# ga1i13o/DiffewS

Hardware: AMD Instinct MI355X
Metric: few-shot episodes/sec (512x512, 1-shot, SD-2 UNet) (higher is better)
Workload: dtype bf16; 1 GPU; SD-2.1 UNet + SD VAE, 512x512, 1-shot, 4 episodes/GPU/step (BASELINE.json configs[1]); nshot=1, resolution=512, parallelism=episode-sharded x1, hip_graph=True, residual_dtype=bf16, graph_owner=pipeline.run_episodes(captured=True)

## Files before the change

diffews_amd/_lib.py:

```python
import ctypes as C
import os

_HERE = os.path.dirname(os.path.abspath(__file__))
LIB_PATH = os.environ.get("DFW_LIB") or os.path.join(_HERE, "libdiffews_hip.so")

BF16, F16 = 0, 1
FILTER_BILINEAR, FILTER_BICUBIC = 0, 1
OUT_T, OUT_F32, OUT_NCHW_F32 = 0, 1, 2
ACT_NONE, ACT_SILU, ACT_CLAMP1 = 0, 1, 2

_vp, _i32, _i64, _f32, _sz = C.c_void_p, C.c_int32, C.c_int64, C.c_float, C.c_size_t


class GemmArgs(C.Structure):
    _fields_ = [("A", _vp), ("W", _vp), ("C", _vp), ("bias", _vp), ("rowbias", _vp), ("residual", _vp),
                ("workspace", _vp), ("workspace_bytes", _sz), ("a_elems", _i64), ("w_elems", _i64),
                ("M", _i32), ("N", _i32), ("K", _i32), ("lda", _i32), ("ldc", _i32), ("ldr", _i32), ("ld_rowbias", _i32),
                ("taps", _i32), ("Cin", _i32), ("Hi", _i32), ("Wi", _i32), ("Ho", _i32), ("Wo", _i32),
                ("stride", _i32), ("pad", _i32), ("ups", _i32), ("rows_per_img", _i32),
                ("out_scale", _f32), ("act", _i32), ("geglu", _i32), ("out_mode", _i32), ("splitk", _i32),
                ("batch", _i32), ("strideA", _i64), ("strideW", _i64), ("strideC", _i64), ("dtype", _i32),
                ("gn_partial", _vp), ("gn_groups", _i32),
                ("colscale", _f32), ("colscale_n", _i32), ("residual_f32", _i32), ("W_blocked", _vp)]


class FsaArgs(C.Structure):
    _fields_ = [("q", _vp), ("k", _vp), ("v", _vp), ("k_bank", _vp), ("v_bank", _vp), ("out", _vp),
                ("batch", _i32), ("heads", _i32), ("n_q", _i32), ("n_kv", _i32), ("n_bank", _i32), ("nshot", _i32),
                ("ldq", _i32), ("ldk", _i32), ("ldv", _i32), ("ldkb", _i32), ("ldvb", _i32), ("ldo", _i32),
                ("q_bs", _i64), ("k_bs", _i64), ("v_bs", _i64), ("kb_bs", _i64), ("vb_bs", _i64), ("o_bs", _i64),
                ("scale", _f32), ("dtype", _i32), ("n_plain", _i32), ("q_prescaled", _i32), ("lse", _vp),
                ("workspace", _vp), ("workspace_bytes", _sz), ("bank_shared", _i32)]


class XattnArgs(C.Structure):
    _fields_ = [("q", _vp), ("k", _vp), ("v", _vp), ("out", _vp),
                ("batch", _i32), ("heads", _i32), ("n_q", _i32), ("L", _i32),
                ("ldq", _i32), ("ldk", _i32), ("ldv", _i32), ("ldo", _i32),
                ("q_bs", _i64), ("k_bs", _i64), ("v_bs", _i64), ("o_bs", _i64),
                ("scale", _f32), ("dtype", _i32)]


class GroupNormArgs(C.Structure):
    _fields_ = [("x", _vp), ("y", _vp), ("gamma", _vp), ("beta", _vp), ("stats_ws", _vp), ("stats_ws_bytes", _sz),
                ("B", _i32), ("HW", _i32), ("C", _i32), ("groups", _i32), ("ldx", _i32), ("ldy", _i32),
                ("eps", _f32), ("silu", _i32), ("dtype", _i32), ("pre_partial", _vp), ("pre_chunks", _i32),
                ("x_f32", _i32)]


class LayerNormArgs(C.Structure):
    _fields_ = [("x", _vp), ("y", _vp), ("gamma", _vp), ("beta", _vp),
                ("rows", _i32), ("C", _i32), ("ldx", _i32), ("ldy", _i32), ("eps", _f32), ("dtype", _i32),
                ("x_f32", _i32)]


class ConvSmallArgs(C.Structure):
    _fields_ = [("x", _vp), ("W", _vp), ("bias", _vp), ("y", _vp),
                ("B", _i32), ("Cin", _i32), ("H", _i32), ("Wd", _i32), ("Cout", _i32), ("taps", _i32), ("ldy", _i32),
                ("in_scale", _f32), ("out_scale", _f32), ("out_mode", _i32), ("dtype", _i32),
                ("gn_partial", _vp), ("gn_groups", _i32), ("y_bstride", _i64),
                ("x1", _vp), ("x2", _vp), ("b0", _i32), ("b1", _i32)]


class ImageArgs(C.Structure):
    _fields_ = [("src", _vp), ("H", _i32), ("W", _i32), ("out_h", _i32), ("out_w", _i32),
                ("xbounds", _vp), ("xcoef", _vp), ("xk", _i32), ("ybounds", _vp), ("ycoef", _vp), ("yk", _i32),
                ("tmp", _vp), ("dst", _vp), ("lut", _vp)]


class NativeItem(C.Structure):
    _fields_ = [("h", _i32), ("w", _i32), ("xk", _i32), ("yk", _i32),
                ("xb_off", _i64), ("xc_off", _i64), ("yb_off", _i64), ("yc_off", _i64),
                ("tmp_off", _i64), ("u8_off", _i64), ("pred_off", _i64), ("gt_off", _i64),
                ("gt_elem", _i32), ("class_value", _i32), ("ignore_value", _i32), ("reserved", _i32)]


class SegNativeArgs(C.Structure):
    _fields_ = [("seg_u8", _vp), ("B", _i32), ("Hs", _i32), ("Ws", _i32), ("items", _vp), ("items_host", _vp),
                ("weights", _vp), ("weights_bytes", _sz), ("gt", _vp), ("gt_bytes", _sz), ("tmp", _vp), ("tmp_bytes", _sz),
                ("tmp_res_off", _sz), ("out_u8", _vp), ("out_u8_bytes", _sz), ("pred", _vp), ("pred_bytes", _sz),
                ("mx", _vp), ("counts", _vp), ("r_threshold", _f32), ("threshold", _f32), ("batch_max", _i32)]


class SegLabelsNativeArgs(C.Structure):
    _fields_ = [("seg_u8", _vp), ("N", _i32), ("B", _i32), ("Hs", _i32), ("Ws", _i32), ("items", _vp), ("items_host", _vp),
                ("weights", _vp), ("weights_bytes", _sz), ("gt", _vp), ("gt_bytes", _sz), ("tmp", _vp), ("tmp_bytes", _sz),
                ("tmp_res_off", _sz), ("tmp_cls_stride", _sz), ("u8_cls_stride", _sz), ("out_u8", _vp), ("out_u8_bytes", _sz),
                ("labels", _vp), ("labels_bytes", _sz), ("mx", _vp), ("counts", _vp), ("class_ids", _vp),
                ("r_threshold", _f32), ("threshold", _f32), ("batch_max", _i32)]


class InputImageItem(C.Structure):
    _fields_ = [("H", _i32), ("W", _i32), ("xk", _i32), ("yk", _i32), ("src_off", _i64),
                ("xb_off", _i64), ("xc_off", _i64), ("yb_off", _i64), ("yc_off", _i64), ("tmp_off", _i64), ("dst_off", _i64)]


class InputMaskItem(C.Structure):
    _fields_ = [("H", _i32), ("W", _i32), ("elem", _i32), ("class_value", _i32),
                ("src_off", _i64), ("pm1_off", _i64), ("bin_off", _i64)]


class InputsArgs(C.Structure):
    _fields_ = [("image_items", _vp), ("image_items_host", _vp), ("n_img", _i32),
                ("mask_items", _vp), ("mask_items_host", _vp), ("n_mask", _i32), ("out_h", _i32), ("out_w", _i32),
                ("staged", _vp), ("staged_bytes", _sz), ("tmp", _vp), ("tmp_bytes", _sz), ("dst", _vp), ("dst_bytes", _sz),
                ("pm1", _vp), ("pm1_bytes", _sz), ("bin", _vp), ("bin_bytes", _sz), ("lut", _vp)]
# ... 41 lines not shown
class AttnBwdArgs(C.Structure):
    _fields_ = [("q", _vp), ("k", _vp), ("v", _vp), ("out", _vp), ("dout", _vp), ("lse", _vp), ("delta", _vp),
                ("dq", _vp), ("dk", _vp), ("dv", _vp),
                ("batch", _i32), ("heads", _i32), ("n_q", _i32), ("n_kv", _i32),
                ("ldq", _i32), ("ldkv", _i32), ("ldo", _i32), ("lddq", _i32), ("lddkv", _i32),
                ("q_bs", _i64), ("kv_bs", _i64), ("o_bs", _i64), ("dq_bs", _i64), ("dkv_bs", _i64),
                ("scale", _f32), ("dtype", _i32), ("workspace", _vp), ("workspace_bytes", _sz), ("delta_bytes", _sz)]


class VattnArgs(C.Structure):
    _fields_ = [("q", _vp), ("k", _vp), ("v", _vp), ("out", _vp),
                ("batch", _i32), ("n", _i32), ("head_dim", _i32), ("q_prescaled", _i32),
                ("ldq", _i32), ("ldk", _i32), ("ldv", _i32), ("ldo", _i32),
                ("q_bs", _i64), ("k_bs", _i64), ("v_bs", _i64), ("o_bs", _i64), ("dtype", _i32)]


class AdamWArgs(C.Structure):
    _fields_ = [("param", _vp), ("grad", _vp), ("exp_avg", _vp), ("exp_avg_sq", _vp), ("grad_sumsq", _vp), ("n", _i64),
                ("lr", _f32), ("beta1", _f32), ("beta2", _f32), ("eps", _f32), ("weight_decay", _f32), ("max_grad_norm", _f32),
                ("step", _i32), ("shadow", _vp), ("shadow_dtype", _i32), ("found_inf", _vp)]


class Config(C.Structure):
    _fields_ = [("conv_patch", _i32), ("big_kernels", _i32), ("big_bm", _i32), ("big_bn", _i32), ("big_bk", _i32),
                ("gemm_bm", _i32), ("gemm_bn", _i32), ("fsa_key_split", _i32),
                ("fsa_force_splits", _i32), ("big_min_tiles", _i32), ("k8", _i32)]


SYMBOLS = {
    "dfw_configure": (_i32, [C.POINTER(Config)]),
    "dfw_get_config": (None, [C.POINTER(Config)]),
    "dfw_version": (_i32, []),
    "dfw_error_string": (C.c_char_p, [_i32]),
    "dfw_graph_memset_nodes": (_i32, [_vp, C.POINTER(_i32)]),
    "dfw_gemm": (_i32, [C.POINTER(GemmArgs), _vp]),
    "dfw_gemm_workspace_bytes": (_sz, [C.POINTER(GemmArgs)]),
    "dfw_gemm_kernel_name": (_i32, [C.POINTER(GemmArgs), C.c_char_p, _sz]),
    "dfw_gemm_gn_chunks": (_i32, [C.POINTER(GemmArgs)]),
    "dfw_fsa_attention": (_i32, [C.POINTER(FsaArgs), _vp]),
    "dfw_fsa_workspace_bytes": (_sz, [C.POINTER(FsaArgs)]),
    "dfw_fsa_kernel_name": (_i32, [C.POINTER(FsaArgs), C.c_char_p, _sz]),
    "dfw_fsa_attention_sets": (_i32, [C.POINTER(FsaArgs), _i32, _vp]),
    "dfw_fsa_sets_kernel_name": (_i32, [C.POINTER(FsaArgs), _i32, C.c_char_p, _sz]),
    "dfw_cross_attention": (_i32, [C.POINTER(XattnArgs), _vp]),
    "dfw_vae_attention": (_i32, [C.POINTER(VattnArgs), _vp]),
    "dfw_groupnorm": (_i32, [C.POINTER(GroupNormArgs), _vp]),
    "dfw_groupnorm_workspace_bytes": (_sz, [C.POINTER(GroupNormArgs)]),
    "dfw_layernorm": (_i32, [C.POINTER(LayerNormArgs), _vp]),
    "dfw_conv_small": (_i32, [C.POINTER(ConvSmallArgs), _vp]),
    "dfw_conv_small_gn_chunks": (_i32, [C.POINTER(ConvSmallArgs)]),
    "dfw_conv_small_kernel_name": (_i32, [C.POINTER(ConvSmallArgs), C.c_char_p, _sz]),
    "dfw_softmax_rows": (_i32, [_vp, _vp, _i64, _i32, _f32, _i32, _vp]),
    "dfw_softmax_groups": (_i32, [_vp, _vp, _i64, _i32, _i32, _i32, _i32, _vp]),
    "dfw_transpose": (_i32, [_vp, _vp, _i32, _i32, _i32, _i32, _vp]),
    "dfw_concat_channels": (_i32, [_vp, _vp, _vp, _i64, _i32, _i32, _i32, _vp]),
    "dfw_convert_f32": (_i32, [_vp, _vp, _i64, _i32, _vp]),
    "dfw_zero": (_i32, [_vp, _i64, _vp]),
    "dfw_split_f32": (_i32, [_vp, _vp, _vp, _i64, _i32, _vp]),
    "dfw_timestep_embedding": (_i32, [_vp, _vp, _i32, _i32, _i32, _f32, _i32, _vp]),
    "dfw_seg_postprocess": (_i32, [_vp, _vp, _vp, _vp, _vp, _i32, _i32, _i32, _f32, _vp]),
    "dfw_seg_postprocess_ex": (_i32, [_vp, _vp, _vp, _vp, _vp, _i32, _i32, _i32, _f32, _f32, _i32, _vp]),
    "dfw_seg_labels": (_i32, [_vp, _vp, _vp, _vp, _vp, _i32, _i32, _i32, _i32, _f32, _f32, _i32, _vp]),
    "dfw_meter_update": (_i32, [_vp, _vp, _vp, _vp, _i32, _i32, _vp]),
    "dfw_gemm_tn": (_i32, [C.POINTER(GemmTnArgs), _vp]),
    "dfw_gemm_tn_workspace_bytes": (_sz, [C.POINTER(GemmTnArgs)]),
    "dfw_gemm_tn_kernel_name": (_i32, [C.POINTER(GemmTnArgs), C.c_char_p, _sz]),
    "dfw_colsum": (_i32, [_vp, _vp, _vp, _sz, _i64, _i32, _i32, _i32, _i64, _f32, _i32, _i32, _vp]),
    "dfw_colsum_plan": (_i32, [_i64, C.POINTER(_i32), C.POINTER(_i32)]),
    "dfw_table_write": (_i32, [_vp, _i64, _vp, _i32, _vp]),
    "dfw_colsum_batch": (_i32, [_vp, _i32, _i64, _i64, _vp, _i32, _vp]),
    "dfw_colsum_workspace_bytes": (_sz, [_i64, _i32, _i32]),
    "dfw_groupnorm_bwd": (_i32, [C.POINTER(GroupNormBwdArgs), _vp]),
    "dfw_groupnorm_bwd_workspace_bytes": (_sz, [C.POINTER(GroupNormBwdArgs)]),
    "dfw_layernorm_bwd": (_i32, [C.POINTER(LayerNormBwdArgs), _vp]),
    "dfw_layernorm_bwd_workspace_bytes": (_sz, [_i32, _i32]),
    "dfw_geglu": (_i32, [_vp, _vp, _vp, _i64, _i32, _i32, _vp]),
    "dfw_elementwise": (_i32, [_i32, _vp, _vp, _vp, _i64, _i32, _i32, _i32, _i32, _i32, _i32, _vp]),
    "dfw_nchw_to_nhwc": (_i32, [_vp, _vp, _i32, _i32, _i32, _i32, _f32, _i32, _vp]),
    "dfw_mse_loss": (_i32, [_vp, _vp, _vp, _vp, _vp, _vp, _i32, _i32, _i32, _f32, _i32, _vp]),
    "dfw_loss_grad": (_i32, [_vp, _vp, _vp, _i32, _i32, _i32, _f32, _i32, _vp]),
    "dfw_convert_to_f32": (_i32, [_vp, _vp, _i64, _f32, _i32, _vp]),
    "dfw_fsa_attention_bwd": (_i32, [C.POINTER(FsaBwdArgs), _vp]),
    "dfw_fsa_attention_bwd_workspace_bytes": (_sz, [C.POINTER(FsaBwdArgs)]),
    "dfw_attention_bwd": (_i32, [C.POINTER(AttnBwdArgs), _vp]),
    "dfw_attention_bwd_workspace_bytes": (_sz, [C.POINTER(AttnBwdArgs)]),
    "dfw_cross_attention_bwd": (_i32, [C.POINTER(XattnBwdArgs), _vp]),
    "dfw_cross_attention_bwd_workspace_bytes": (_sz, [_i32, _i32, _i32, _i32]),
    "dfw_silu": (_i32, [_vp, _vp, _vp, _i64, _i32, _vp]),
    "dfw_sumsq": (_i32, [_vp, _vp, _vp, _i64, _vp]),
    "dfw_adamw": (_i32, [C.POINTER(AdamWArgs), _vp]),
    "dfw_weight_relayout": (_i32, [_vp, _vp, _i32, _i32, _i64, _i64, _i32, _i64, _i64, _i32, _vp]),
    "dfw_weight_relayout_batch": (_i32, [_vp, _i32, _i64, _vp]),
    "dfw_resample_ksize": (_i32, [_i32, _i32]),
    "dfw_resample_coeffs": (_i32, [_i32, _i32, _vp, _vp]),
    "dfw_image_to_tensor": (_i32, [C.POINTER(ImageArgs), _vp]),
    "dfw_mask_to_tensor": (_i32, [_vp, _i32, _i32, _i32, _i32, _i32, _i32, _vp, _vp, _vp]),
    "dfw_resample_ksize_ex": (_i32, [_i32, _i32, _i32]),
    "dfw_resample_coeffs_ex": (_i32, [_i32, _i32, _i32, _vp, _vp]),
    "dfw_seg_native": (_i32, [C.POINTER(SegNativeArgs), _vp]),
    "dfw_seg_labels_native": (_i32, [C.POINTER(SegLabelsNativeArgs), _vp]),
    "dfw_inputs_to_tensor": (_i32, [C.POINTER(InputsArgs), _vp]),
}

_lib = None


# ... 37 lines not shown
```

diffews_amd/build.py:

```python
import os
import subprocess
import sys

HERE = os.path.dirname(os.path.abspath(__file__))
CSRC = os.path.join(HERE, "csrc")
LIB = os.path.join(HERE, "libdiffews_hip.so")
SOURCES = ["gemm.hip", "gemm_big.hip", "gemm8.hip", "conv_patch.hip", "conv_patch8.hip", "attention.hip", "vae_attention.hip", "attention_bwd.hip", "backward.hip", "norm.hip",
           "misc.hip", "inputs.hip", "seg_native.hip"]
FLAGS = ["--offload-arch=gfx950", "-O3", "-std=c++17", "-fPIC", "-ffp-contract=fast", "-Wno-unused-result", "-Wno-unused-value"]


def _src_hash():
    import hashlib
    h = hashlib.sha256(" ".join(FLAGS).encode())
    deps = sorted(os.path.join(CSRC, f) for f in os.listdir(CSRC)) + [os.path.join(HERE, "..", "include", "diffews_hip.h")]
    for d in deps:
        with open(d, "rb") as f:
            h.update(os.path.basename(d).encode() + b"\0" + f.read())
    return h.hexdigest()


def _stale():
    if not os.path.isfile(LIB) or not os.path.isfile(LIB + ".srchash"):
        return True
    with open(LIB + ".srchash") as f:
        return f.read().strip() != _src_hash()


def build(force=False, verbose=False):
    if not force and not _stale():
        return LIB
    if os.environ.get("DFW_NO_BUILD"):
        raise RuntimeError(f"{LIB} is missing or older than its sources and DFW_NO_BUILD is set: "
                           "run `python -m diffews_amd.build` first")
    hipcc = os.environ.get("HIPCC", "hipcc")
    objs = []
    procs = []
    os.makedirs(os.path.join(HERE, "build"), exist_ok=True)
    for src in SOURCES:
        obj = os.path.join(HERE, "build", src.replace(".hip", ".o"))
        objs.append(obj)
        cmd = [hipcc, *FLAGS, "-c", os.path.join(CSRC, src), "-o", obj]
        if verbose:
            print(" ".join(cmd), flush=True)
        procs.append((src, subprocess.Popen(cmd, stdout=subprocess.PIPE, stderr=subprocess.STDOUT, text=True)))
    for src, pr in procs:
        out, _ = pr.communicate()
        if pr.returncode != 0:
            raise RuntimeError(f"hipcc failed for {src}:\n{out}")
        if verbose and out.strip():
            print(out)
    cmd = [hipcc, "--offload-arch=gfx950", "-shared", "-fPIC", "-o", LIB, *objs]
    r = subprocess.run(cmd, stdout=subprocess.PIPE, stderr=subprocess.STDOUT, text=True)
    if r.returncode != 0:
        raise RuntimeError(f"link failed:\n{r.stdout}")
    with open(LIB + ".srchash", "w") as f:
        f.write(_src_hash())
    return LIB


if __name__ == "__main__":
# ... 2 lines not shown
```

diffews_amd/ops.py:

```python
import ctypes as C
import os
import math

import torch

from . import _lib as L

_DT = {torch.bfloat16: L.BF16, torch.float16: L.F16}


def _stream():
    return C.c_void_p(torch.cuda.current_stream().cuda_stream)


def _p(t):
    return C.c_void_p(t.data_ptr()) if t is not None else None


def _dt(t):
    try:
        return _DT[t.dtype]
    except KeyError:
        raise TypeError(f"engine storage dtype must be bfloat16 or float16, got {t.dtype}")

# ... 357 lines not shown
    a.in_scale, a.out_scale = in_scale, out_scale
    a.out_mode = L.OUT_NCHW_F32 if nchw_f32_out else (L.OUT_F32 if out_f32 else L.OUT_T)
    a.dtype = _DT[dtype]
    stats = None
    if gn_groups and not nchw_f32_out and not out_f32:
        a.gn_groups = gn_groups
        chunks = L.lib().dfw_conv_small_gn_chunks(C.byref(a))
        if chunks > 0:
            part = gn_part if gn_part is not None else torch.empty(B, chunks, gn_groups, 2, dtype=torch.float32, device=x.device)
            assert part.shape == (B, chunks, gn_groups, 2) and part.is_contiguous() and part.dtype == torch.float32
            a.gn_partial = part.data_ptr()
            stats = (part, chunks, gn_groups)
    L.check(L.lib().dfw_conv_small(C.byref(a), _stream()), "dfw_conv_small")
    if stats is not None:
        y._gn_stats = stats
    return y


def conv_small_gn_chunks(x_shape, cout, taps, dtype, gn_groups):
    B, Cin, H, W = x_shape
    a = L.ConvSmallArgs()
    a.B, a.Cin, a.H, a.Wd, a.Cout, a.taps, a.ldy = B, Cin, H, W, cout, taps, cout
    a.out_mode, a.dtype, a.gn_groups = L.OUT_T, _DT[dtype], gn_groups
    a.x = 16
    return L.lib().dfw_conv_small_gn_chunks(C.byref(a))


def meter_update(counts, class_id, inter_buf, union_buf):
    assert counts.dtype == torch.int64 and counts.is_contiguous() and counts.shape[1] == 4
    assert class_id.dtype == torch.int64 and class_id.is_contiguous() and class_id.shape[0] == counts.shape[0]
    assert inter_buf.dtype == torch.int64 and inter_buf.is_contiguous() and union_buf.is_contiguous()
    L.check(L.lib().dfw_meter_update(counts.data_ptr(), class_id.data_ptr(), inter_buf.data_ptr(), union_buf.data_ptr(),
                                     counts.shape[0], inter_buf.shape[1], _stream()), "dfw_meter_update")


def softmax_rows(x, dtype, scale=1.0):
    assert x.dtype == torch.float32 and x.is_contiguous()
    Lr = x.shape[-1]
    rows = x.numel() // Lr
    y = torch.empty(x.shape, dtype=dtype, device=x.device)
    L.check(L.lib().dfw_softmax_rows(x.data_ptr(), y.data_ptr(), rows, Lr, scale, _DT[dtype], _stream()),
            "dfw_softmax_rows")
    return y


def softmax_groups(x, groups, L_, dtype):
    assert x.dtype == torch.float32 and x.dim() == 2 and x.is_contiguous()
    y = torch.empty(x.shape, dtype=dtype, device=x.device)
    L.check(L.lib().dfw_softmax_groups(x.data_ptr(), y.data_ptr(), x.shape[0], x.shape[1], groups, L_,
                                       _DT[dtype], _stream()), "dfw_softmax_groups")
    return y


def transpose(x):
    assert x.dim() == 3 and x.is_contiguous()
    Bt, R, Cc = x.shape
    y = torch.empty(Bt, Cc, R, dtype=x.dtype, device=x.device)
    L.check(L.lib().dfw_transpose(x.data_ptr(), y.data_ptr(), Bt, R, Cc, _dt(x), _stream()), "dfw_transpose")
    return y


def concat_channels(a, b):
    assert a.is_contiguous() and b.is_contiguous() and a.shape[:-1] == b.shape[:-1] and a.dtype == b.dtype
    Ca, Cb = a.shape[-1], b.shape[-1]
    y = torch.empty(*a.shape[:-1], Ca + Cb, dtype=a.dtype, device=a.device)
    rows = a.numel() // Ca
    if a.dtype == torch.float32:
        L.check(L.lib().dfw_concat_channels(a.data_ptr(), b.data_ptr(), y.data_ptr(), rows, 2 * Ca, 2 * Cb, L.BF16, _stream()),
                "dfw_concat_channels")
        return y
    L.check(L.lib().dfw_concat_channels(a.data_ptr(), b.data_ptr(), y.data_ptr(), rows, Ca, Cb, _dt(a), _stream()),
            "dfw_concat_channels")
    return y


def to_storage(x, dtype):
    if x.dtype == dtype:
        return x
    assert x.dtype == torch.float32 and x.is_contiguous() and x.numel() % 8 == 0
    y = torch.empty(x.shape, dtype=dtype, device=x.device)
    L.check(L.lib().dfw_convert_f32(x.data_ptr(), y.data_ptr(), x.numel(), _DT[dtype], _stream()), "dfw_convert_f32")
    return y


def timestep_embedding(timesteps, dim, dtype, flip_sin_to_cos=True, freq_shift=0.0):
    assert timesteps.dtype == torch.float32 and timesteps.is_contiguous() and timesteps.dim() == 1
    out = torch.empty(timesteps.shape[0], dim, dtype=dtype, device=timesteps.device)
    L.check(L.lib().dfw_timestep_embedding(timesteps.data_ptr(), out.data_ptr(), timesteps.shape[0], dim,
                                           int(flip_sin_to_cos), float(freq_shift), _DT[dtype], _stream()),
            "dfw_timestep_embedding")
    return out


def seg_postprocess(x, gt=None, r_threshold=0.25, threshold=0.0, batch_max=False, u8_out=None, counts_out=None,
                    scratch=None):
    assert x.dtype == torch.float32 and x.is_contiguous() and x.dim() == 4 and x.shape[1] == 3
    B, _, H, W = x.shape
    u8 = u8_out if u8_out is not None else torch.empty(B, 3, H, W, dtype=torch.uint8, device=x.device)
    if scratch is None:
        scratch = torch.empty(B, dtype=torch.int32, device=x.device)
    counts = None
    if gt is not None:
        assert gt.dtype == torch.uint8 and gt.is_contiguous() and gt.shape == (B, H, W)
        counts = counts_out if counts_out is not None else torch.empty(B, 4, dtype=torch.int64, device=x.device)
    L.check(L.lib().dfw_seg_postprocess_ex(x.data_ptr(), u8.data_ptr(), _p(gt), _p(counts), scratch.data_ptr(),
                                           B, H, W, float(r_threshold), float(threshold), int(bool(batch_max)),
# ... 115 lines not shown
```

diffews_amd/unet.py:

```python
from dataclasses import dataclass

import os

import torch

from . import _lib as L
from . import ops, ops_bwd, packing, weights


@dataclass
class UNet2DConditionOutput:
    sample: torch.Tensor = None


class _Cfg(dict):
    __getattr__ = dict.__getitem__


def _resolve_device(d):
    d = torch.device(d)
    if d.type == "cuda" and d.index is None:
        d = torch.device("cuda", torch.cuda.current_device() if torch.cuda.is_available() else 0)
    return d

# ... 162 lines not shown
        if not banks:
            raise ValueError("support bank set: stack() of no banks")
        b0 = banks[0]
        for i, b in enumerate(banks[1:], 1):
            for name, attr in (("nshot", "nshot"), ("latent (h, w)", "hw"), ("storage dtype", "dtype"),
                               ("residual-stream dtype", "residual_dtype"), ("fold key (timestep, prompt)", "fold_key"),
                               ("weights", "weights_id")):
                if getattr(b, attr) != getattr(b0, attr):
                    raise ValueError(f"support bank set: bank {i} differs from bank 0 in {name}: {getattr(b, attr)} "
                                     f"against {getattr(b0, attr)}")
        n = len(b0.k)
        k = [torch.cat([b.k[i] for b in banks], 0) for i in range(n)]
        v = [torch.cat([b.v[i] for b in banks], 0) for i in range(n)]
        layout = [tuple(t.shape[1:]) for t in b0.k]
        return SupportBankSet(k, v, len(banks), b0.nshot, b0.hw, b0.dtype, b0.residual_dtype, b0.fold_key, b0.weights_id,
                              layout)


class _BankIO:

    def __init__(self, n, bank=None, k=None, v=None, group=0):
        self.fill = bank is None
        self.k = [None] * n if bank is None else (bank.k if k is None else k)
        self.v = [None] * n if bank is None else (bank.v if v is None else v)
        self.nshot = 0 if bank is None else bank.nshot
        self.group = group


class _Transformer:

    def __init__(self, sd, p, dev, dt, heads, groups):
        g = lambda k: sd[p + k]
        f = lambda k: g(k).float().to(dev)
        w = lambda k: g(k).to(dev, dt).contiguous()
        self.heads, self.groups = heads, groups
        self.gn_g, self.gn_b = f("norm.weight"), f("norm.bias")
        self.w_in, self.b_in = w("proj_in.weight"), f("proj_in.bias")
        self.w_out, self.b_out = w("proj_out.weight"), f("proj_out.bias")
        b = "transformer_blocks.0."
        self.ln = [(f(b + n + ".weight"), f(b + n + ".bias")) for n in ("norm1", "norm2", "norm3")]
        self.w_qkv = torch.cat([g(b + "attn1.to_q.weight"), g(b + "attn1.to_k.weight"),
                                g(b + "attn1.to_v.weight")], 0).to(dev, dt).contiguous()
        self.w_o1, self.b_o1 = w(b + "attn1.to_out.0.weight"), f(b + "attn1.to_out.0.bias")
        self.w_q2 = w(b + "attn2.to_q.weight")
        self.w_kv2 = torch.cat([g(b + "attn2.to_k.weight"), g(b + "attn2.to_v.weight")], 0).to(dev, dt).contiguous()
        self.w_o2, self.b_o2 = w(b + "attn2.to_out.0.weight"), f(b + "attn2.to_out.0.bias")
        wp, bp = packing.pack_geglu(g(b + "ff.net.0.proj.weight"), g(b + "ff.net.0.proj.bias"))
        self.w_ff1, self.b_ff1 = wp.to(dev, dt), bp.to(dev)
        self.w_ff2, self.b_ff2 = w(b + "ff.net.2.weight"), f(b + "ff.net.2.bias")
        self.k_bank = None
        self.v_bank = None
        self.kv_slice = (0, 2 * self.w_q2.shape[0])
        self.fold2 = None
        self.index = 0

    def fold_attn2(self, kv, L_ctx):
        C, h = self.w_q2.shape[0], self.heads
        if h * L_ctx > 64:
            self.fold2 = None
            return
        dev = kv.device
        kv = kv.float().cpu()
        k, v = kv[:, :C], kv[:, C:2 * C]
        wq, wo = self.w_q2.float().cpu(), self.w_o2.float().cpu()
        G = torch.zeros(64, C, dtype=torch.float32)
        Ut = torch.zeros(C, 64, dtype=torch.float32)
        for hh in range(h):
            blk = slice(hh * 64, (hh + 1) * 64)
            G[hh * L_ctx:(hh + 1) * L_ctx] = (64 ** -0.5) * (k[:, blk] @ wq[blk, :])
            Ut[:, hh * L_ctx:(hh + 1) * L_ctx] = wo[:, blk] @ v[:, blk].t()
        self.fold2 = (G.to(dev, self.w_q2.dtype).contiguous(), Ut.to(dev, self.w_q2.dtype).contiguous(), L_ctx)

    def clear_bank(self):
        self.k_bank = None
        self.v_bank = None

    def __call__(self, x, ehs2d, L_ctx, n_ref=0, bank_io=None):
        B, H, W, C = x.shape
        N = H * W
        heads = self.heads
        dt, f32s = self.w_in.dtype, x.dtype == torch.float32
        n = ops.groupnorm(x, self.gn_g, self.gn_b, self.groups, 1e-6, silu=False, out_dtype=dt)
        t = ops.linear(n.view(-1, C), self.w_in, bias=self.b_in, out_f32=f32s)
        ln = ops.layernorm(t, *self.ln[0], out_dtype=dt)
        qkv = ops.linear(ln, self.w_qkv, colscale=(C, ops.FSA_QSCALE)).view(B, N, 3 * C)
        q, k, v = qkv[..., :C], qkv[..., C:2 * C], qkv[..., 2 * C:]
        if bank_io is not None and bank_io.fill:
            kv = ops_bwd.slice_channels(qkv, C, 2 * C)
            bank_io.k[self.index], bank_io.v[self.index] = kv[..., :C], kv[..., C:]
            att = ops.fsa_attention(q, k, v, heads, q_prescaled=True)
        elif bank_io is not None and bank_io.group:
            att = ops.fsa_attention_sets(q, k, v, heads, bank_io.k[self.index], bank_io.v[self.index], bank_io.nshot,
                                         bank_io.group, q_prescaled=True)
        elif bank_io is not None:
            att = ops.fsa_attention(q, k, v, heads, bank_io.k[self.index], bank_io.v[self.index], nshot=bank_io.nshot,
                                    q_prescaled=True, bank_shared=True)
        elif n_ref:
            bq = B - n_ref
            if bq <= 0 or n_ref % bq != 0:
                raise ValueError(f"{n_ref} support images is not a multiple of the {bq} query images")
            att = ops.fsa_attention(q, k, v, heads, k[:n_ref], v[:n_ref], nshot=n_ref // bq, n_plain=n_ref,
                                    q_prescaled=True)
        elif self.k_bank is None:
            self.k_bank, self.v_bank = k, v
            att = ops.fsa_attention(q, k, v, heads, q_prescaled=True)
        else:
            bank_b = self.k_bank.shape[0]
            if bank_b % B != 0:
                raise ValueError(f"bank holds {bank_b} support images, not a multiple of the query batch {B}")
            att = ops.fsa_attention(q, k, v, heads, self.k_bank, self.v_bank, nshot=bank_b // B, q_prescaled=True)
        t = ops.linear(att.view(-1, C), self.w_o1, bias=self.b_o1, residual=t, out_f32=f32s)
        ln = ops.layernorm(t, *self.ln[1], out_dtype=dt)
        if isinstance(ehs2d, tuple) and len(ehs2d) == 3 and ehs2d[2] and self.fold2 is not None:
            G, Ut, Lf = self.fold2
            sc = ops.linear(ln, G, out_f32=True)
            pr = ops.softmax_groups(sc, heads, Lf, dt)
            t = ops.linear(pr, Ut, bias=self.b_o2, residual=t, out_f32=f32s)
        else:
            q2 = ops.linear(ln, self.w_q2).view(B, N, C)
            o, kv_all = self.kv_slice[0], ehs2d
            if isinstance(kv_all, tuple):
                kv2 = kv_all[1].view(B, L_ctx, -1)[..., o:o + 2 * C]
            else:
                kv2 = ops.linear(ehs2d, self.w_kv2).view(B, L_ctx, 2 * C)
            ca = ops.cross_attention(q2, kv2[..., :C], kv2[..., C:], heads)
            t = ops.linear(ca.view(-1, C), self.w_o2, bias=self.b_o2, residual=t, out_f32=f32s)
        ln = ops.layernorm(t, *self.ln[2], out_dtype=dt)
        ff = ops.linear(ln, self.w_ff1, bias=self.b_ff1, geglu=True)
        t = ops.linear(ff, self.w_ff2, bias=self.b_ff2, residual=t, out_f32=f32s)
        return ops.linear_stream(t, self.w_out, bias=self.b_out, residual=x.view(-1, C)).view(B, H, W, C)


class _Conv:
    def __init__(self, sd, p, dev, dt):
        self.w = packing.pack_conv3x3(sd[p + "weight"]).to(dev, dt)
        self.b = sd[p + "bias"].float().to(dev)
        self.cout = sd[p + "weight"].shape[0]


class MyUNet2DConditionModel:

    def __init__(self, config=None, state_dict=None, torch_dtype=torch.bfloat16, device="cuda", residual_dtype=None,
                 **kwargs):
        cfg = weights.default_unet_config()
        cfg.update(config or {})
        cfg.update(kwargs)
        self.config = _Cfg(cfg)
        if residual_dtype not in (None, torch_dtype, torch.float32):
            raise ValueError("residual_dtype must be None (= torch_dtype) or torch.float32")
        self.residual_dtype = residual_dtype or torch_dtype
        self._f32s = self.residual_dtype == torch.float32
        if torch_dtype not in (torch.bfloat16, torch.float16):
            raise ValueError(
                "engine storage dtype must be torch.bfloat16 or torch.float16: the MI355X path keeps activations in 16 bits "
                "(fp32 accumulation, statistics and boundary tensors).  The reference launcher's default is fp32 "
                "(evaluation_util/main_oss.py:335-336): pass --half_precision / torch_dtype=torch.float16 -- z0 then sits "
                "1.5e-3 (relative L2) from the fp32 path, see DESIGN.md section 4")
        self.dtype = torch_dtype
        self.device = torch.device(device)
        L.lib()
        if state_dict is None:
            raise ValueError("MyUNet2DConditionModel needs a state_dict (use from_pretrained / synthetic weights)")
        weights.check_state_dict(state_dict, weights.unet_param_shapes(cfg), "unet")
        self._build(state_dict)

    @classmethod
# ... 349 lines not shown
```

include/diffews_hip.h:

```cpp
#ifndef DIFFEWS_HIP_H
#define DIFFEWS_HIP_H

#include <stddef.h>
#include <stdint.h>

#ifdef __cplusplus
extern "C" {
#endif

typedef void* dfw_stream_t;

enum { DFW_BF16 = 0, DFW_F16 = 1 };
enum { DFW_OUT_T = 0, DFW_OUT_F32 = 1, DFW_OUT_NCHW_F32 = 2 };
enum { DFW_ACT_NONE = 0, DFW_ACT_SILU = 1, DFW_ACT_CLAMP1 = 2  };
enum {
  DFW_EINVAL = -1,
  DFW_ESHAPE = -2,
  DFW_ERANGE = -3,
  DFW_EWORKSPACE = -4
};

int dfw_version(void);
const char* dfw_error_string(int code);

// ... 65 lines not shown
  int64_t q_bs, k_bs, v_bs, o_bs;
  float scale;
  int32_t dtype;
} dfw_xattn_args;

int dfw_cross_attention(const dfw_xattn_args* a, dfw_stream_t stream);

typedef struct {
  const void* x; void* y; const float* gamma; const float* beta;
  void* stats_ws; size_t stats_ws_bytes;
  int32_t B, HW, C, groups, ldx, ldy;
  float eps;
  int32_t silu;
  int32_t dtype;
  const float* pre_partial; int32_t pre_chunks;
  int32_t x_f32;
} dfw_groupnorm_args;

int dfw_groupnorm(const dfw_groupnorm_args* a, dfw_stream_t stream);
size_t dfw_groupnorm_workspace_bytes(const dfw_groupnorm_args* a);

typedef struct {
  const void* x; void* y; const float* gamma; const float* beta;
  int32_t rows, C, ldx, ldy;
  float eps;
  int32_t dtype;
  int32_t x_f32;
} dfw_layernorm_args;

int dfw_layernorm(const dfw_layernorm_args* a, dfw_stream_t stream);

typedef struct {
  const float* x; const float* W; const float* bias; void* y;
  int32_t B, Cin, H, Wd, Cout, taps, ldy;
  float in_scale, out_scale;
  int32_t out_mode;
  int32_t dtype;
  float* gn_partial; int32_t gn_groups;
  int64_t y_bstride;
  const float* x1; const float* x2; int32_t b0, b1;
} dfw_conv_small_args;

int dfw_conv_small(const dfw_conv_small_args* a, dfw_stream_t stream);
int32_t dfw_conv_small_gn_chunks(const dfw_conv_small_args* a);
int dfw_conv_small_kernel_name(const dfw_conv_small_args* a, char* buf, size_t n);

int dfw_softmax_rows(const float* x, void* y, int64_t rows, int32_t L, float scale, int32_t dtype,
                     dfw_stream_t stream);

int dfw_softmax_groups(const float* x, void* y, int64_t rows, int32_t ld, int32_t groups, int32_t L,
                       int32_t dtype, dfw_stream_t stream);
int dfw_transpose(const void* x, void* y, int32_t batch, int32_t R, int32_t C, int32_t dtype,
                  dfw_stream_t stream);

int dfw_concat_channels(const void* a, const void* b, void* y, int64_t rows, int32_t Ca, int32_t Cb,
                        int32_t dtype, dfw_stream_t stream);

int dfw_convert_f32(const float* x, void* y, int64_t n, int32_t dtype, dfw_stream_t stream);

int dfw_zero(void* p, int64_t bytes, dfw_stream_t stream);

int dfw_split_f32(const float* x, void* hi, void* lo, int64_t n, int32_t dtype, dfw_stream_t stream);

int dfw_timestep_embedding(const float* timesteps, void* out, int32_t B, int32_t dim,
                           int32_t flip_sin_to_cos, float freq_shift, int32_t dtype,
                           dfw_stream_t stream);

int dfw_seg_postprocess(const float* x, uint8_t* seg_u8, const uint8_t* gt, int64_t* counts,
                        uint32_t* scratch, int32_t B, int32_t H, int32_t Wd, float r_threshold,
                        dfw_stream_t stream);
int dfw_seg_postprocess_ex(const float* x, uint8_t* seg_u8, const uint8_t* gt, int64_t* counts,
                           uint32_t* scratch, int32_t B, int32_t H, int32_t Wd, float r_threshold,
                           float threshold, int32_t batch_max, dfw_stream_t stream);

int dfw_seg_labels(const uint8_t* seg_u8, const uint32_t* mx, const uint8_t* gt, uint8_t* labels, int64_t* counts,
                   int32_t N, int32_t B, int32_t H, int32_t Wd, float r_threshold, float threshold,
                   int32_t batch_max, dfw_stream_t stream);

int dfw_meter_update(const int64_t* counts, const int64_t* class_id, int64_t* inter_buf, int64_t* union_buf,
                     int32_t B, int32_t nclass, dfw_stream_t stream);

int32_t dfw_resample_ksize(int32_t in_size, int32_t out_size);
int dfw_resample_coeffs(int32_t in_size, int32_t out_size, int32_t* bounds, int32_t* coeffs);

typedef struct {
  const uint8_t* src;
  int32_t H, W, out_h, out_w;
  const int32_t* xbounds; const int32_t* xcoef; int32_t xk;
  const int32_t* ybounds; const int32_t* ycoef; int32_t yk;
  uint8_t* tmp;
  float* dst;
  const float* lut;
} dfw_image_args;

int dfw_image_to_tensor(const dfw_image_args* a, dfw_stream_t stream);
int dfw_mask_to_tensor(const void* mask, int32_t elem_bytes, int32_t H, int32_t W, int32_t class_value,
                       int32_t out_h, int32_t out_w, float* dst_pm1, uint8_t* dst_bin, dfw_stream_t stream);

enum { DFW_FILTER_BILINEAR = 0, DFW_FILTER_BICUBIC = 1 };
int32_t dfw_resample_ksize_ex(int32_t in_size, int32_t out_size, int32_t filter);
int dfw_resample_coeffs_ex(int32_t in_size, int32_t out_size, int32_t filter, int32_t* bounds, int32_t* coeffs);

typedef struct {
  int32_t h, w;
  int32_t xk, yk;
  int64_t xb_off, xc_off;
// ... 234 lines not shown
```

Before: 102.2 episodes/s.

## Fuse layernorm, folded cross-attention scores, softmax and output projection into one kernel

Adds a HIP kernel that computes layernorm of the residual stream, the folded cross-attention score GEMM against G, the grouped softmax, the projection through Ut, bias and residual add in one pass per 16-row tile. This replaces four separate launches and their intermediate tensor round-trips (ln, fp32 scores, probabilities) in every transformer block's attn2 when the context is folded. In exchange it adds an LDS cross-wave reduction, keeps larger register footprints for wide channel counts, and is limited to bf16/fp16 with C up to 1280 and heads*L up to 64.

New measurement: 102.6 episodes/s (median of 6 runs). No clear change (+0.4%).

```diff
diff --git a/diffews_amd/_lib.py b/diffews_amd/_lib.py
--- a/diffews_amd/_lib.py
+++ b/diffews_amd/_lib.py
@@ -52,6 +52,11 @@
     _fields_ = [("x", _vp), ("y", _vp), ("gamma", _vp), ("beta", _vp),
                 ("rows", _i32), ("C", _i32), ("ldx", _i32), ("ldy", _i32), ("eps", _f32), ("dtype", _i32),
                 ("x_f32", _i32)]
+
+
+class Attn2FoldedArgs(C.Structure):
+    _fields_ = [("t", _vp), ("out", _vp), ("gamma", _vp), ("beta", _vp), ("G", _vp), ("Ut", _vp), ("bias", _vp),
+                ("M", _i32), ("C", _i32), ("heads", _i32), ("L", _i32), ("eps", _f32), ("dtype", _i32)]
 
 
 class ConvSmallArgs(C.Structure):
@@ -199,6 +204,8 @@
     "dfw_conv_small_kernel_name": (_i32, [C.POINTER(ConvSmallArgs), C.c_char_p, _sz]),
     "dfw_softmax_rows": (_i32, [_vp, _vp, _i64, _i32, _f32, _i32, _vp]),
     "dfw_softmax_groups": (_i32, [_vp, _vp, _i64, _i32, _i32, _i32, _i32, _vp]),
+    "dfw_attn2_folded": (_i32, [C.POINTER(Attn2FoldedArgs), _vp]),
+    "dfw_attn2_folded_ok": (_i32, [_i32, _i32, _i32, _i32]),
     "dfw_transpose": (_i32, [_vp, _vp, _i32, _i32, _i32, _i32, _vp]),
     "dfw_concat_channels": (_i32, [_vp, _vp, _vp, _i64, _i32, _i32, _i32, _vp]),
     "dfw_convert_f32": (_i32, [_vp, _vp, _i64, _i32, _vp]),
diff --git a/diffews_amd/build.py b/diffews_amd/build.py
--- a/diffews_amd/build.py
+++ b/diffews_amd/build.py
@@ -6,7 +6,7 @@
 CSRC = os.path.join(HERE, "csrc")
 LIB = os.path.join(HERE, "libdiffews_hip.so")
 SOURCES = ["gemm.hip", "gemm_big.hip", "gemm8.hip", "conv_patch.hip", "conv_patch8.hip", "attention.hip", "vae_attention.hip", "attention_bwd.hip", "backward.hip", "norm.hip",
-           "misc.hip", "inputs.hip", "seg_native.hip"]
+           "misc.hip", "inputs.hip", "seg_native.hip", "attn2_folded.hip"]
 FLAGS = ["--offload-arch=gfx950", "-O3", "-std=c++17", "-fPIC", "-ffp-contract=fast", "-Wno-unused-result", "-Wno-unused-value"]
 
 
diff --git a/diffews_amd/csrc/attn2_folded.hip b/diffews_amd/csrc/attn2_folded.hip
--- /dev/null
+++ b/diffews_amd/csrc/attn2_folded.hip
@@ -0,0 +1,218 @@
+#include "common.h"
+
+namespace dfw {
+
+struct A2P {
+  const char* t; char* out; const float* gamma; const float* beta; const char* G; const char* Ut; const float* bias;
+  int M, C, heads, L;
+  float eps;
+};
+
+template <int L>
+__device__ __forceinline__ void softmax4(const f32x4 x, int q0, int nvalid, float* p) {
+#pragma unroll
+  for (int g = 0; g < 4; g += L) {
+    float m = x[g];
+#pragma unroll
+    for (int l = 1; l < L; ++l) m = fmaxf(m, x[g + l]);
+    float sum = 0.f;
+#pragma unroll
+    for (int l = 0; l < L; ++l) sum += __expf(x[g + l] - m);
+    const float inv = 1.0f / sum;
+    const bool ok = q0 + g < nvalid;
+#pragma unroll
+    for (int l = 0; l < L; ++l) p[g + l] = ok ? __expf(x[g + l] - m) * inv : 0.f;
+  }
+}
+
+template <typename T, int NW, int NSW>
+__global__ __launch_bounds__(NW * 64) void attn2_folded_kernel(const A2P p) {
+  using v8 = typename Tr<T>::v8;
+  __shared__ float red[2][NW][16];
+  __shared__ f32x4 part[NW][4][64];
+  const int lane = threadIdx.x & 63, w = threadIdx.x >> 6, r = lane & 15, q = lane >> 4;
+  const int row = blockIdx.x * 16 + r;
+  const bool live = row < p.M;
+  const int ns = p.C >> 5;
+  const size_t rowb = (size_t)p.C * sizeof(T);
+  const char* tr = p.t + (size_t)row * rowb + q * 16;
+
+  i32x4 raw[NSW];
+#pragma unroll
+  for (int i = 0; i < NSW; ++i) {
+    const int s = w + i * NW;
+    raw[i] = i32x4{0, 0, 0, 0};
+    if (s < ns && live) raw[i] = *(const i32x4*)(tr + s * 64);
+  }
+  v8 ga[NSW][4];
+#pragma unroll
+  for (int i = 0; i < NSW; ++i) {
+    const int s = w + i * NW;
+#pragma unroll
+    for (int b = 0; b < 4; ++b) {
+      ga[i][b] = as_v8<T>(i32x4{0, 0, 0, 0});
+      if (s < ns)
+        ga[i][b] = as_v8<T>(*(const i32x4*)(p.G + (size_t)(32 * (b >> 1) + 8 * (r >> 2) + 4 * (b & 1) + (r & 3)) * rowb + q * 16 + s * 64));
+    }
+  }
+
+  float sum = 0.f;
+#pragma unroll
+  for (int i = 0; i < NSW; ++i) {
+    float f[8];
+    unpack8<T>(raw[i], f);
+#pragma unroll
+    for (int j = 0; j < 8; ++j) sum += f[j];
+  }
+  sum += __shfl_xor(sum, 16, 64);
+  sum += __shfl_xor(sum, 32, 64);
+  if (q == 0) red[0][w][r] = sum;
+  __syncthreads();
+  sum = 0.f;
+#pragma unroll
+  for (int k = 0; k < NW; ++k) sum += red[0][k][r];
+  const float mean = sum / p.C;
+  float var = 0.f;
+#pragma unroll
+  for (int i = 0; i < NSW; ++i)
+    if (w + i * NW < ns) {
+      float f[8];
+      unpack8<T>(raw[i], f);
+#pragma unroll
+      for (int j = 0; j < 8; ++j) { const float d = f[j] - mean; var += d * d; }
+    }
+  var += __shfl_xor(var, 16, 64);
+  var += __shfl_xor(var, 32, 64);
+  if (q == 0) red[1][w][r] = var;
+  __syncthreads();
+  var = 0.f;
+#pragma unroll
+  for (int k = 0; k < NW; ++k) var += red[1][k][r];
+  const float rstd = rsqrtf(var / p.C + p.eps);
+
+  f32x4 sc[4];
+#pragma unroll
+  for (int b = 0; b < 4; ++b) sc[b] = f32x4{0.f, 0.f, 0.f, 0.f};
+#pragma unroll
+  for (int i = 0; i < NSW; ++i) {
+    const int s = w + i * NW;
+    if (s < ns) {
+      const int c0 = 32 * s + 8 * q;
+      const f32x4 g0 = *(const f32x4*)(p.gamma + c0), g1 = *(const f32x4*)(p.gamma + c0 + 4);
+      const f32x4 b0 = *(const f32x4*)(p.beta + c0), b1 = *(const f32x4*)(p.beta + c0 + 4);
+      float f[8], o[8];
+      unpack8<T>(raw[i], f);
+#pragma unroll
+      for (int j = 0; j < 4; ++j) {
+        o[j] = (f[j] - mean) * rstd * g0[j] + b0[j];
+        o[4 + j] = (f[4 + j] - mean) * rstd * g1[j] + b1[j];
+      }
+      const v8 ln = as_v8<T>(pack8<T>(o));
+#pragma unroll
+      for (int b = 0; b < 4; ++b) sc[b] = Tr<T>::mfma16(ga[i][b], ln, sc[b]);
+    }
+  }
+  const char* ufrag = p.Ut + (size_t)(8 * (r >> 2) + (r & 3)) * 128 + q * 16;
+  v8 ua[NSW][2][2];
+#pragma unroll
+  for (int i = 0; i < NSW; ++i) {
+    const int s = w + i * NW;
+#pragma unroll
+    for (int h = 0; h < 2; ++h)
+#pragma unroll
+      for (int k2 = 0; k2 < 2; ++k2) {
+        ua[i][h][k2] = as_v8<T>(i32x4{0, 0, 0, 0});
+        if (s < ns) ua[i][h][k2] = as_v8<T>(*(const i32x4*)(ufrag + (size_t)(32 * s + 4 * h) * 128 + k2 * 64));
+      }
+  }
+#pragma unroll
+  for (int b = 0; b < 4; ++b) part[w][b][lane] = sc[b];
+  __syncthreads();
+#pragma unroll
+  for (int b = 0; b < 4; ++b) {
+    sc[b] = part[0][b][lane];
+#pragma unroll
+    for (int k = 1; k < NW; ++k) sc[b] += part[k][b][lane];
+  }
+
+  const int nvalid = p.heads * p.L;
+  v8 pr[2];
+#pragma unroll
+  for (int k2 = 0; k2 < 2; ++k2) {
+    float pf[8];
+#pragma unroll
+    for (int h = 0; h < 2; ++h) {
+      const int q0 = 32 * k2 + 8 * q + 4 * h;
+      if (p.L == 1) softmax4<1>(sc[2 * k2 + h], q0, nvalid, pf + 4 * h);
+      else if (p.L == 2) softmax4<2>(sc[2 * k2 + h], q0, nvalid, pf + 4 * h);
+      else softmax4<4>(sc[2 * k2 + h], q0, nvalid, pf + 4 * h);
+    }
+    pr[k2] = as_v8<T>(pack8<T>(pf));
+  }
+
+  char* orow = p.out + (size_t)row * rowb + q * 16;
+#pragma unroll
+  for (int i = 0; i < NSW; ++i) {
+    const int s = w + i * NW;
+    if (s < ns) {
+      f32x4 acc[2];
+#pragma unroll
+      for (int h = 0; h < 2; ++h) {
+        acc[h] = Tr<T>::mfma16(ua[i][h][0], pr[0], f32x4{0.f, 0.f, 0.f, 0.f});
+        acc[h] = Tr<T>::mfma16(ua[i][h][1], pr[1], acc[h]);
+      }
+      const int c0 = 32 * s + 8 * q;
+      const f32x4 bi0 = *(const f32x4*)(p.bias + c0), bi1 = *(const f32x4*)(p.bias + c0 + 4);
+      float f[8], o[8];
+      unpack8<T>(raw[i], f);
+#pragma unroll
+      for (int j = 0; j < 4; ++j) {
+        o[j] = acc[0][j] + bi0[j] + f[j];
+        o[4 + j] = acc[1][j] + bi1[j] + f[4 + j];
+      }
+      if (live) *(i32x4*)(orow + s * 64) = pack8<T>(o);
+    }
+  }
+}
+
+}
+
+using namespace dfw;
+
+extern "C" int dfw_attn2_folded_ok(int32_t C, int32_t heads, int32_t L, int32_t dtype) {
+  if (dtype != DFW_BF16 && dtype != DFW_F16) return 0;
+  if (C < 64 || C > 1280 || C % 64 != 0) return 0;
+  if (L != 1 && L != 2 && L != 4) return 0;
+  if (heads < 1 || heads * L > 64) return 0;
+  return 1;
+}
+
+template <typename T>
+static void launch_attn2_folded(const A2P& p, hipStream_t st) {
+  const dim3 grid((p.M + 15) / 16);
+  const int ns = p.C / 32;
+  if (ns <= 4) hipLaunchKernelGGL((attn2_folded_kernel<T, 4, 1>), grid, dim3(256), 0, st, p);
+  else if (ns <= 12) hipLaunchKernelGGL((attn2_folded_kernel<T, 4, 3>), grid, dim3(256), 0, st, p);
+  else if (ns <= 20) hipLaunchKernelGGL((attn2_folded_kernel<T, 4, 5>), grid, dim3(256), 0, st, p);
+  else hipLaunchKernelGGL((attn2_folded_kernel<T, 8, 5>), grid, dim3(512), 0, st, p);
+}
+
+extern "C" int dfw_attn2_folded(const dfw_attn2_folded_args* a, dfw_stream_t stream) {
+  if (!a) return DFW_EINVAL;
+  if (a->dtype != DFW_BF16 && a->dtype != DFW_F16) return DFW_EINVAL;
+  if (a->M <= 0) return DFW_EINVAL;
+  if (!dfw_attn2_folded_ok(a->C, a->heads, a->L, a->dtype)) return DFW_ESHAPE;
+  if (!a->t || !a->out || !a->gamma || !a->beta || !a->G || !a->Ut || !a->bias || a->t == a->out) return DFW_EINVAL;
+  if ((((uintptr_t)a->t | (uintptr_t)a->out | (uintptr_t)a->gamma | (uintptr_t)a->beta | (uintptr_t)a->G | (uintptr_t)a->Ut |
+        (uintptr_t)a->bias) & 15) != 0)
+    return DFW_EINVAL;
+  A2P p;
+  p.t = (const char*)a->t; p.out = (char*)a->out; p.gamma = a->gamma; p.beta = a->beta;
+  p.G = (const char*)a->G; p.Ut = (const char*)a->Ut; p.bias = a->bias;
+  p.M = a->M; p.C = a->C; p.heads = a->heads; p.L = a->L; p.eps = a->eps;
+  hipStream_t st = (hipStream_t)stream;
+  if (a->dtype == DFW_BF16) launch_attn2_folded<__bf16>(p, st);
+  else launch_attn2_folded<_Float16>(p, st);
+  DFW_CHECK_LAUNCH();
+  return 0;
+}
diff --git a/diffews_amd/ops.py b/diffews_amd/ops.py
--- a/diffews_amd/ops.py
+++ b/diffews_amd/ops.py
@@ -433,6 +433,24 @@
     return y
 
 
+def attn2_folded_ok(C_, heads, L_, dtype):
+    return dtype in _DT and bool(L.lib().dfw_attn2_folded_ok(C_, heads, L_, _DT[dtype]))
+
+
+def attn2_folded(t, gamma, beta, G, Ut, bias, heads, L_, eps=1e-5):
+    assert t.dim() == 2 and t.is_contiguous() and t.dtype in _DT
+    M, C_ = t.shape
+    assert G.shape == (64, C_) and Ut.shape == (C_, 64) and G.is_contiguous() and Ut.is_contiguous()
+    assert G.dtype == t.dtype and Ut.dtype == t.dtype
+    out = torch.empty_like(t)
+    a = L.Attn2FoldedArgs()
+    a.t, a.out, a.G, a.Ut = t.data_ptr(), out.data_ptr(), G.data_ptr(), Ut.data_ptr()
+    a.gamma, a.beta, a.bias = _p(_f32(gamma, "gamma")), _p(_f32(beta, "beta")), _p(_f32(bias, "bias"))
+    a.M, a.C, a.heads, a.L, a.eps, a.dtype = M, C_, heads, L_, eps, _DT[t.dtype]
+    L.check(L.lib().dfw_attn2_folded(C.byref(a), _stream()), "dfw_attn2_folded")
+    return out
+
+
 def transpose(x):
     assert x.dim() == 3 and x.is_contiguous()
     Bt, R, Cc = x.shape
diff --git a/diffews_amd/unet.py b/diffews_amd/unet.py
--- a/diffews_amd/unet.py
+++ b/diffews_amd/unet.py
@@ -238,6 +238,7 @@
         self.v_bank = None
         self.kv_slice = (0, 2 * self.w_q2.shape[0])
         self.fold2 = None
+        self.fuse_attn2 = True
         self.index = 0
 
     def fold_attn2(self, kv, L_ctx):
@@ -296,8 +297,13 @@
                 raise ValueError(f"bank holds {bank_b} support images, not a multiple of the query batch {B}")
             att = ops.fsa_attention(q, k, v, heads, self.k_bank, self.v_bank, nshot=bank_b // B, q_prescaled=True)
         t = ops.linear(att.view(-1, C), self.w_o1, bias=self.b_o1, residual=t, out_f32=f32s)
-        ln = ops.layernorm(t, *self.ln[1], out_dtype=dt)
-        if isinstance(ehs2d, tuple) and len(ehs2d) == 3 and ehs2d[2] and self.fold2 is not None:
+        folded = isinstance(ehs2d, tuple) and len(ehs2d) == 3 and ehs2d[2] and self.fold2 is not None
+        fused = folded and self.fuse_attn2 and not f32s and ops.attn2_folded_ok(C, heads, self.fold2[2], dt)
+        ln = None if fused else ops.layernorm(t, *self.ln[1], out_dtype=dt)
+        if fused:
+            G, Ut, Lf = self.fold2
+            t = ops.attn2_folded(t, *self.ln[1], G, Ut, self.b_o2, heads, Lf)
+        elif folded:
             G, Ut, Lf = self.fold2
             sc = ops.linear(ln, G, out_f32=True)
             pr = ops.softmax_groups(sc, heads, Lf, dt)
diff --git a/include/diffews_hip.h b/include/diffews_hip.h
--- a/include/diffews_hip.h
+++ b/include/diffews_hip.h
@@ -141,6 +141,16 @@
                        int32_t dtype, dfw_stream_t stream);
 int dfw_transpose(const void* x, void* y, int32_t batch, int32_t R, int32_t C, int32_t dtype,
                   dfw_stream_t stream);
+
+typedef struct {
+  const void* t; void* out; const float* gamma; const float* beta; const void* G; const void* Ut; const float* bias;
+  int32_t M, C, heads, L;
+  float eps;
+  int32_t dtype;
+} dfw_attn2_folded_args;
+
+int dfw_attn2_folded(const dfw_attn2_folded_args* a, dfw_stream_t stream);
+int dfw_attn2_folded_ok(int32_t C, int32_t heads, int32_t L, int32_t dtype);
 
 int dfw_concat_channels(const void* a, const void* b, void* y, int64_t rows, int32_t Ca, int32_t Cb,
                         int32_t dtype, dfw_stream_t stream);
```
